# CloudEngineHub/PARC

Measured on AMD Instinct MI355X. Metric: env-steps/s, higher is better.
Workload: dtype f32; 1 GPU; full step (dynamics + obs/reward/done), 65536 envs total = 65536 per GPU, 5 bundled clips on a square blocky grid, reset of finished envs included; envs_per_gpu=65536, total_envs=65536, dynamics=True, parallelism=env-shard x1, launch=stream launches, library_abi=6

## Files before the change

### parc_amd/csrc/parc_env.hip

```cpp
#include <hip/hip_runtime.h>

#include <cmath>
#include <cstddef>
#include <cstdio>
#include <cstring>
#include <memory>
#include <new>
#include <string>
#include <type_traits>
#include <vector>

#include "../../include/parc_env.h"
#include "parc_common.hpp"
#include "parc_math.hpp"
#include "parc_rowmap.hpp"
#include "parc_lanetab.hpp"
#include "parc_dynamics.hpp"
#include "parc_dynamics_coop.hpp"
#include "parc_dynamics_wave.hpp"

using namespace parc;

#define REC_F4 32
#define REC_Q_POS 15
#define REC_Q_CONTACT 16
#define REC_Q_VEL 20

struct HierTables {
    float lt[16][3];
    float lr[16][4];
    int fk_paths[PARC_MAX_FK_PATHS][PARC_MAX_FK_DEPTH];
    int key_ids[8];
    int key_slot[16];
    int parent[16];
    int jtype[16];
    int dof_idx[16];
    float axis[16][4];
};
#define HIER_STAGED_WORDS ((int)(offsetof(HierTables, parent) / 4))

#define TILE_MAX_CELLS 320

struct DevTables {
    HierTables h;
    float tstep[8];
    float joint_err_w[16];
    float dof_err_w[PARC_MAX_DOFS];
    float contact_w[16];
    float pose_term_dist[16];
    ParcLaneEntry lane[64];
};

struct StepParams {
    int N, B, J, D, K, S, R, M, T;
    int lds_wave_floats;
    int global_obs, off_char;
    int lr_identity;
    int obs_tar, obs_contact;
    int obs_dim, off_dofvel, off_key, off_tar, tar_w, off_tarc, off_cc, off_hf;
    float dt_f, episode_length, min_obs_h, max_obs_h;
    float pose_w, vel_w, root_pos_w, root_vel_w, key_pos_w;
    float root_pos_term_sq, root_rot_term;
    int early_term, pose_term, track_root, track_root_h, tracking, body_pos_from_fk, never_done;
    unsigned fall_mask;
    float term_h;
    const float *hf; int X, Y; float min_x, min_y, dx, dy; int tile_r;
    float rdx, rdy;
    float tstep[8];
    const float4 *records; const MotionMeta *meta; const float *motion_offsets; const float *env_offsets;
    const float *ray_points; const DevTables *tables;
    unsigned char *ema_code;
    unsigned *stamp_out;
    float4 *prep;
    ParcEnvBuffers buf;
};

__device__ __forceinline__ Q4 joint_dof_to_rot(int type, const float *axis4, const float *dof) {
    if (type == PARC_JOINT_HINGE) return axis_angle_to_quat(mk3(axis4[0], axis4[1], axis4[2]), dof[0]);
    if (type == PARC_JOINT_SPHERICAL) return exp_map_to_quat(mk3(dof[0], dof[1], dof[2]));
    return mk4(0.f, 0.f, 0.f, 1.f);
}

__device__ __forceinline__ void joint_rot_to_dof(int type, const float *axis4, Q4 q, float *out) {
// ... 69 lines not shown
#endif
#define MODE_STEP 0
#define MODE_OBS 1
#define ENVS_PER_BLOCK 4
#define WAVE_SYNC() asm volatile("" ::: "memory")
#define RAY_UNROLL 8

__device__ __forceinline__ float wave_sum(float v) {
#pragma unroll
    for (int off = 32; off >= 1; off >>= 1) v = v + __shfl_xor(v, off, 64);
    return v;
}

template <int CTRL>
__device__ __forceinline__ float dpp_f32(float v) {
    return __int_as_float(__builtin_amdgcn_update_dpp(0, __float_as_int(v), CTRL, 0xf, 0xf, false));
}
__device__ __forceinline__ float row_sum16(float v) {
    v = v + dpp_f32<0x128>(v);
    v = v + dpp_f32<0x124>(v);
    v = v + dpp_f32<0x122>(v);
    v = v + dpp_f32<0x121>(v);
    return v;
}
__device__ __forceinline__ float lane_value(float v, int l) { return __int_as_float(__builtin_amdgcn_readlane(__float_as_int(v), l)); }

template <int MODE, bool MIRROR, bool LOCALROOT = false, bool OBSVAR = false>
__global__ __launch_bounds__(256, 5) void k_env_post(const StepParams P, const int64_t *__restrict__ env_ids,
                                                 const int *__restrict__ env_ids32, const int *__restrict__ count_dev, int count,
                                                 unsigned long long *bump_calls) {
    extern __shared__ __align__(16) float s_obs_all[];
    __shared__ int s_tab_raw[HIER_STAGED_WORDS];
    const HierTables &s_tab = *reinterpret_cast<const HierTables *>(s_tab_raw);
    __shared__ float4 s_q_all[ENVS_PER_BLOCK][8][16];
    __shared__ float4 s_lq_all[ENVS_PER_BLOCK][2][16];
    __shared__ float4 s_fk_all[ENVS_PER_BLOCK][80];
    __shared__ float s_cdofv_all[ENVS_PER_BLOCK][PARC_MAX_DOFS];
    __shared__ float4 s_refvel_all[ENVS_PER_BLOCK][12];
    __shared__ float s_refct_all[ENVS_PER_BLOCK][16];
    __shared__ float s_cfn_all[ENVS_PER_BLOCK][16];
    __shared__ float s_sc_all[ENVS_PER_BLOCK][16];
#ifdef PARC_STAMPS
    __shared__ unsigned long long s_stamp_all[ENVS_PER_BLOCK][16];
#endif
    const int wv = __builtin_amdgcn_readfirstlane((int)(threadIdx.x >> 6));
    const int lane = threadIdx.x & 63;
    const bool GLOBALOBS = OBSVAR && P.global_obs != 0;
    const int oc = OBSVAR ? P.off_char : 0;
    const bool TAROBS = !OBSVAR || P.obs_tar != 0;
    const bool CONTACTOBS = !OBSVAR || P.obs_contact != 0;
    float *s_obs = s_obs_all + (size_t)wv * P.lds_wave_floats;
    float4 (*s_q)[16] = s_q_all[wv];
    float4 (*s_lq)[16] = s_lq_all[wv];
    float4 *s_fk = s_fk_all[wv];
    float4 *s_cbp = s_lq[0];
    float *s_cdofv = s_cdofv_all[wv];
    float4 *s_refvel = s_refvel_all[wv];
    float *s_refct = s_refct_all[wv], *s_cfn = s_cfn_all[wv];
#ifdef PARC_STAMPS
    unsigned long long *s_stamp = s_stamp_all[wv];
#endif
    float *s_tile = (float *)s_fk;
    float4 (*s_br)[16] = reinterpret_cast<float4 (*)[16]>(s_obs + ((P.off_tarc + 3) & ~3));

    if (MODE == MODE_OBS && bump_calls && blockIdx.x == 0 && threadIdx.x == 0) *bump_calls += 1ull;
    if (count_dev) count = *count_dev;
    const int it = blockIdx.x * ENVS_PER_BLOCK + wv;
    if (it >= count) return;
    int e = env_ids ? (int)env_ids[it] : (env_ids32 ? env_ids32[it] : it);
    e = __builtin_amdgcn_readfirstlane(e);
    STAMP(0);

    const int B = P.B, D = P.D, S = P.S, K = P.K, J = P.J;
    const DevTables *__restrict__ T = P.tables;

    float *orow = P.buf.obs + (size_t)e * P.obs_dim;

    constexpr int HW = HIER_STAGED_WORDS;
    constexpr int HN = (HW + 63) / 64;
    int tabreg[HN];
#pragma unroll
    for (int i = 0; i < HN; ++i) { const int w = lane + 64 * i; tabreg[i] = w < HW ? ((const int *)&T->h)[w] : 0; }
    unsigned lt[PARC_LANETAB_WORDS];
    {
        static_assert(sizeof(ParcLaneEntry) == sizeof(uint4), "one 16-byte load per lane");
        const uint4 l0 = *reinterpret_cast<const uint4 *>(T->lane + lane);
        lt[0] = l0.x; lt[1] = l0.y; lt[2] = l0.z; lt[3] = l0.w;
// ... 24 lines not shown
    const float time = P.dt_f * (float)ts;
    const float mt = time + toff;
    const MotionMeta meta = P.meta[mid];
    const float eox = P.env_offsets[3 * e + 0], eoy = P.env_offsets[3 * e + 1], eoz = P.env_offsets[3 * e + 2];
    const float *mo = P.motion_offsets + 2 * ((size_t)mid * P.T + tid);
    const float offx = mo[0] - eox, offy = mo[1] - eoy;
    const float *crp = P.buf.char_root_pos + 3 * (size_t)e;
    const float *crr = P.buf.char_root_rot + 4 * (size_t)e;
    const V3 root_pos = mk3(crp[0], crp[1], crp[2]);
    const Q4 root_rot = mk4(crr[0], crr[1], crr[2], crr[3]);
    const float gx = root_pos.x + eox, gy = root_pos.y + eoy, gz = root_pos.z + eoz;

    Blend myb;
    {
        const int sid = lane & 7;
        float t = mt;
#pragma unroll
        for (int q = 0; q < PARC_MAX_TAR_STEPS; ++q) t = (sid - 1 == q) ? mt + P.tstep[q] : t;
        myb = frame_blend(meta, t);
    }
    const int last_frame = meta.start + meta.nframes - 1;
    float4 fA[2], fB[2];
    Blend bl[2];
#pragma unroll
    for (int p = 0; p < 2; ++p) {
        const int src4 = (int)parc_lt_src4(lt, p);
        bl[p].b = __int_as_float(__builtin_amdgcn_ds_bpermute(src4, __float_as_int(myb.b)));
        bl[p].i0 = __builtin_amdgcn_ds_bpermute(src4, myb.i0);
        bl[p].i1 = min(bl[p].i0 + 1, last_frame);
        const unsigned slot = parc_lt_row_slot(lt, p);
        fA[p] = P.records[(size_t)bl[p].i0 * REC_F4 + slot];
        fB[p] = P.records[(size_t)bl[p].i1 * REC_F4 + slot];
    }
    const int nvel = 2 + (D + 3) / 4;
    const int src4c = (int)parc_lt_src4(lt, 2);
    const float cblend = __int_as_float(__builtin_amdgcn_ds_bpermute(src4c, __float_as_int(myb.b)));
    const int b2i0 = __builtin_amdgcn_ds_bpermute(src4c, myb.i0), b2i1 = min(b2i0 + 1, last_frame);
    const float4 cA = P.records[(size_t)b2i0 * REC_F4 + parc_lt_cv_slot0(lt)];
    const float4 cB = P.records[(size_t)b2i1 * REC_F4 + parc_lt_cv_slot1(lt)];
    static_assert(64 * PARC_LANETAB_TILE_CELLS == TILE_MAX_CELLS && TILE_MAX_CELLS * sizeof(float) == sizeof(s_fk_all[0]), "the five tile stores of a lane stay inside s_fk");
    const int tr = P.tile_r, TW = 2 * tr + 1;
    const int ox = min(max(cell_index(gx, P.min_x, P.dx) - tr, -(1 << 22)), 1 << 22), oy = min(max(cell_index(gy, P.min_y, P.dy) - tr, -(1 << 22)), 1 << 22);
    float tilev[5];
#pragma unroll
    for (int i = 0; i < 5; ++i) {
        const int cx = min(max(ox + (int)parc_lt_cell_a(lt, i), 0), P.X - 1), cy = min(max(oy + (int)parc_lt_cell_b(lt, i), 0), P.Y - 1);
        tilev[i] = P.hf[(size_t)cx * P.Y + cy];
    }

    const float ch = __shfl(prepq.x, 0, 64), sh = __shfl(prepq.y, 0, 64);
    const Q4 hinv = mk4(0.f, 0.f, __shfl(prepq.z, 0, 64), __shfl(prepq.w, 0, 64));
#pragma unroll
    for (int i = 0; i < HN; ++i) { const int w = lane + 64 * i; if (w < HW) s_tab_raw[w] = tabreg[i]; }
    if (lane < D) {
        s_cdofv[lane] = dofv;
        s_obs[P.off_dofvel + lane] = dofv;
    }
    if (OBSVAR && oc && lane == 29) s_obs[0] = root_pos.z;
    if (role == PARC_LT_ROLE_ROOT_VEL || role == PARC_LT_ROLE_ROOT_ANG_VEL) {
        const V3 r = GLOBALOBS ? mk3(aux0, aux1, aux2) : quat_rotate(hinv, mk3(aux0, aux1, aux2));
        const int o = oc + (role == PARC_LT_ROLE_ROOT_VEL ? 6 : 9);
        s_obs[o + 0] = r.x; s_obs[o + 1] = r.y; s_obs[o + 2] = r.z;
    }
    if (role == PARC_LT_ROLE_FORCE) {
        const float n = norm3(mk3(aux0, aux1, aux2));
        if (CONTACTOBS) orow[P.off_cc + (lane - 32)] = n > 1e-5f ? 1.f : 0.f;
        s_cfn[lane - 32] = fminf(n, 1.0f);
    }
#pragma unroll
    for (int i = 0; i < 5; ++i) s_tile[lane + 64 * i] = tilev[i];
    WAVE_SYNC();
    STAMP(1);

    {
        float *hrow = orow + P.off_hf;
        float *hmirror = MIRROR && P.buf.ray_hfs ? P.buf.ray_hfs + (size_t)e * P.R : nullptr;
        for (int base = 0; base < P.R; base += 64 * RAY_UNROLL) {
            if (base > 0) {
#pragma unroll
                for (int i = 0; i < RAY_UNROLL; ++i) { const int r = base + lane + 64 * i; rayp[i] = r < P.R ? ((const float2 *)P.ray_points)[r] : make_float2(0.f, 0.f); }
            }
            const float tlox = (float)ox, thix = (float)(ox + TW - 1), tloy = (float)oy, thiy = (float)(oy + TW - 1);
            if (tr >= 0) {
                int tix[RAY_UNROLL];
#pragma unroll
                for (int i = 0; i < RAY_UNROLL; ++i) {
                    tix[i] = 0;
                    if (base + 64 * i < P.R) {
                        const float px = (rayp[i].x * ch - rayp[i].y * sh) + gx;
                        const float py = (rayp[i].x * sh + rayp[i].y * ch) + gy;
                        const int a = (int)fminf(fmaxf(cell_float_rcp(px, P.min_x, P.dx, P.rdx), tlox), thix) - ox;
                        const int bq = (int)fminf(fmaxf(cell_float_rcp(py, P.min_y, P.dy, P.rdy), tloy), thiy) - oy;
                        tix[i] = a * TW + bq;
                    }
                    asm volatile("" : "+v"(tix[i]));
                }
// ... 1 lines not shown
#pragma unroll
                for (int i = 0; i < RAY_UNROLL; ++i) hv[i] = s_tile[tix[i]];
#pragma unroll
                for (int i = 0; i < RAY_UNROLL; ++i) {
                    const int r = base + lane + 64 * i;
                    if (r < P.R) {
                        float h = hv[i] - gz;
                        h = fminf(fmaxf(h, P.min_obs_h), P.max_obs_h);
                        hrow[r] = h;
                        if (hmirror) hmirror[r] = h;
                    }
                }
            } else {
#pragma unroll
                for (int i = 0; i < RAY_UNROLL; ++i) {
                    const int r = base + lane + 64 * i;
                    if (r < P.R) {
                        const float px = (rayp[i].x * ch - rayp[i].y * sh) + gx;
                        const float py = (rayp[i].x * sh + rayp[i].y * ch) + gy;
                        const int ix = cell_index_rcp(px, P.min_x, P.dx, P.rdx), iy = cell_index_rcp(py, P.min_y, P.dy, P.rdy);
                        const int cx = min(max(ix, 0), P.X - 1), cy = min(max(iy, 0), P.Y - 1);
                        float h = P.hf[(size_t)cx * P.Y + cy] - gz;
                        h = fminf(fmaxf(h, P.min_obs_h), P.max_obs_h);
                        hrow[r] = h;
                        if (hmirror) hmirror[r] = h;
                    }
                }
            }
        }
    }
    STAMP(2);

    static_assert(2 * (PARC_MAX_BODIES - 2) <= PARC_ROWMAP_JOINTS_A, "the joints of rows 0 and 1 must fit into pass A");
    auto row_pass = [&](auto root_tag, const int itm, const float4 A, const float4 Bv, const float bb) {
        constexpr bool ROOT = decltype(root_tag)::value;
        if (itm < 0) return;
        const int r = itm >> 4, i = itm & 15;
        const bool is_rot = ROOT && i == 0, is_pos = ROOT && i == 15;
        const bool row0 = ROOT && r == 0, row1 = ROOT && r == 1;
        float4 res = make_float4(0.f, 0.f, 0.f, 1.f);
        if (row0) {
            if (is_rot) res = root_rot;
            else if (is_pos) res = make_float4(root_pos.x, root_pos.y, root_pos.z, 0.f);
            else res = prepq;
        } else {
            if (is_pos) {
                const float a = 1.0f - bb;
                res.x = a * A.x + bb * Bv.x;
                res.y = a * A.y + bb * Bv.y;
                res.z = a * A.z + bb * Bv.z;
                res.w = 0.f;
                if (meta.loop == PARC_LOOP_WRAP) {
                    float t = mt;
#pragma unroll
                    for (int q = 0; q < PARC_MAX_TAR_STEPS; ++q) t = (r - 2 == q) ? mt + P.tstep[q] : t;
                    const float ph = floorf(t / meta.length);
                    res.x = res.x + ph * meta.dx; res.y = res.y + ph * meta.dy; res.z = res.z + ph * meta.dz;
                }
                res.x = res.x + offx;
                res.y = res.y + offy;
            } else {
                res = slerp_rr(A, Bv, bb);
            }
        }
        if (!is_rot && !is_pos) {
            const Q4 lq = P.lr_identity ? res : quat_mul(mk4(s_tab.lr[i][0], s_tab.lr[i][1], s_tab.lr[i][2], s_tab.lr[i][3]), res);
            if (row0 || row1) { s_lq[r][i] = lq; s_q[r][i] = res; } else s_q[r][i] = lq;
        } else {
            s_q[r][i] = res;
        }
        if (row1) {
            if (MIRROR && is_rot && P.buf.ref_root_rot) *(float4 *)(P.buf.ref_root_rot + 4 * (size_t)e) = res;
            if (MIRROR && !is_rot && !is_pos && P.buf.ref_joint_rot) *(float4 *)(P.buf.ref_joint_rot + 4 * ((size_t)e * J + i - 1)) = res;
            if (MIRROR && is_pos && P.buf.ref_root_pos) {
                float *o = P.buf.ref_root_pos + 3 * (size_t)e;
                o[0] = res.x; o[1] = res.y; o[2] = res.z;
            }
        } else if (row0 || TAROBS) {
            const int base = row0 ? 0 : P.off_tar + (r - 2) * P.tar_w;
            if (!is_pos) {
                const Q4 qq = (is_rot && !GLOBALOBS) ? quat_mul(hinv, res) : res;
                float tn[6];
                quat_to_tan_norm(qq, tn);
                const int o = row0 ? oc + (is_rot ? 0 : 12 + 6 * (i - 1)) : base + 3 + 6 * i;
#pragma unroll
                for (int c = 0; c < 6; ++c) s_obs[o + c] = tn[c];
            } else if (!row0) {
                const V3 rpd = mk3(res.x - root_pos.x, res.y - root_pos.y, res.z - root_pos.z);
                const V3 rpo = GLOBALOBS ? rpd : quat_rotate(hinv, rpd);
                s_obs[base + 0] = rpo.x; s_obs[base + 1] = rpo.y; s_obs[base + 2] = rpo.z;
            }
        }
    };
    row_pass(std::true_type(), item[0], fA[0], fB[0], bl[0].b);
    row_pass(std::false_type(), item[1], fA[1], fB[1], bl[1].b);
    if (lane < 4 * (1 + S)) {
        const int s = lane >> 2, c = lane & 3;
        const float b = cblend, a = 1.0f - b;
        const float v[4] = {a * cA.x + b * cB.x, a * cA.y + b * cB.y, a * cA.z + b * cB.z, a * cA.w + b * cB.w};
#pragma unroll
        for (int k = 0; k < 4; ++k) {
            const int bd = 4 * c + k;
            if (bd < B) {
                if (s == 0) {
                    s_refct[bd] = v[k];
                    if (MIRROR && P.buf.ref_contacts) P.buf.ref_contacts[(size_t)e * B + bd] = v[k];
                } else if (TAROBS && CONTACTOBS) {
                    orow[P.off_tarc + (s - 1) * B + bd] = v[k];
                }
            }
        }
    } else if (lane >= 32 && lane < 32 + nvel) {
        const int c = lane - 32;
        s_refvel[c] = cA;
        if (MIRROR && c == 0 && P.buf.ref_root_vel) { float *o = P.buf.ref_root_vel + 3 * (size_t)e; o[0] = cA.x; o[1] = cA.y; o[2] = cA.z; }
        if (MIRROR && c == 1 && P.buf.ref_root_ang_vel) { float *o = P.buf.ref_root_ang_vel + 3 * (size_t)e; o[0] = cA.x; o[1] = cA.y; o[2] = cA.z; }
        if (MIRROR && c >= 2 && P.buf.ref_dof_vel) {
            const float vv[4] = {cA.x, cA.y, cA.z, cA.w};
            for (int k = 0; k < 4; ++k) { const int d = 4 * (c - 2) + k; if (d < D) P.buf.ref_dof_vel[(size_t)e * D + d] = vv[k]; }
        }
    }
    float bpx = 0.f, bpy = 0.f, bpz = 0.f;
    if (!P.body_pos_from_fk && lane < B) {
        const float *src = P.buf.char_body_pos + 3 * ((size_t)e * B + lane);
        bpx = src[0]; bpy = src[1]; bpz = src[2];
    }
    WAVE_SYNC();
    STAMP(3);

    {
        const int k = lane >> 3, c = lane & 7;
        if (k < 2 + S) {
            Q4 prot = s_q[k][0];
            const float4 *jq = k < 2 ? s_lq[k] : s_q[k];
            const float4 pp = s_q[k][15];
            V3 ppos = mk3(pp.x, pp.y, pp.z);
            if (c == 0 && k < 2) {
                s_fk[k * 16] = make_float4(ppos.x, ppos.y, ppos.z, 0.f);
                if (MIRROR && P.tracking) s_br[k][0] = prot;
            }
            int b = s_tab.fk_paths[c][0];
#pragma unroll 1
            for (int d = 0; d < PARC_MAX_FK_DEPTH && b >= 0; ++d) {
                const int nb = d + 1 < PARC_MAX_FK_DEPTH ? s_tab.fk_paths[c][d + 1] : -1;
                const V3 wt = quat_rotate(prot, mk3(s_tab.lt[b][0], s_tab.lt[b][1], s_tab.lt[b][2]));
                ppos = mk3(ppos.x + wt.x, ppos.y + wt.y, ppos.z + wt.z);
                if (nb >= 0 || (MIRROR && P.tracking)) prot = quat_mul(prot, jq[b]);
                if (k < 2) {
                    s_fk[k * 16 + b] = make_float4(ppos.x, ppos.y, ppos.z, 0.f);
                    if (MIRROR && P.tracking) s_br[k][b] = prot;
                } else {
                    const int slot = s_tab.key_slot[b];
                    if (slot >= 0) s_fk[32 + (k - 2) * 8 + slot] = make_float4(ppos.x, ppos.y, ppos.z, 0.f);
                }
                b = nb;
            }
        }
    }
    WAVE_SYNC();
    if (lane < B) s_cbp[lane] = P.body_pos_from_fk ? s_fk[lane] : make_float4(bpx, bpy, bpz, 0.f);
    STAMP(4);

    if (lane < 8 * (1 + S)) {
        const int row = lane >> 3, kk = lane & 7;
        if (kk < K) {
            if (row == 0) {
                const float4 kp = s_fk[s_tab.key_ids[kk]];
                const V3 rd = mk3(kp.x - root_pos.x, kp.y - root_pos.y, kp.z - root_pos.z);
                const V3 rl = GLOBALOBS ? rd : quat_rotate(hinv, rd);
                const int o = P.off_key + 3 * kk;
                s_obs[o] = rl.x; s_obs[o + 1] = rl.y; s_obs[o + 2] = rl.z;
            } else if (TAROBS) {
                const int r = row + 1;
                const float4 kp = s_fk[32 + (r - 2) * 8 + s_tab.key_slot[s_tab.key_ids[kk]]], trp = s_q[r][15];
                const V3 rd = mk3(kp.x - trp.x, kp.y - trp.y, kp.z - trp.z);
                const int tb = P.off_tar + (r - 2) * P.tar_w, o = tb + 3 + 6 * B + 3 * kk;
                if (GLOBALOBS) {
                    s_obs[o] = rd.x; s_obs[o + 1] = rd.y; s_obs[o + 2] = rd.z;
                } else {
                    const V3 rl = quat_rotate(hinv, rd);
                    s_obs[o] = rl.x + s_obs[tb]; s_obs[o + 1] = rl.y + s_obs[tb + 1]; s_obs[o + 2] = rl.z + s_obs[tb + 2];
                }
            }
        }
    }
    STAMP(5);

    if (MODE == MODE_STEP) {
        {
            float *sc = s_sc_all[wv];
            bool fc = false;
            if (P.fall_mask != 0u && lane >= 32 && lane < 32 + B && !((P.fall_mask >> (lane - 32)) & 1u))
                fc = fabsf(aux0) > 0.1f || fabsf(aux1) > 0.1f || fabsf(aux2) > 0.1f;
            const bool fcany = __ballot(fc) != 0ull;
            if (lane == 30) { sc[5] = aux0; sc[6] = aux1; sc[7] = aux2; }
            if (lane == 31) { sc[8] = aux0; sc[9] = aux1; sc[10] = aux2; }
            if (lane == 0) {
                sc[0] = time; sc[1] = mt; sc[2] = __int_as_float(ts); sc[3] = meta.length; sc[4] = __int_as_float(meta.loop);
                sc[11] = fcany ? 1.f : 0.f; sc[12] = eox; sc[13] = eoy; sc[14] = __int_as_float(e);
            }
        }
        asm volatile("s_waitcnt lgkmcnt(0)\n\ts_barrier" ::: "memory");
        const int nact = min(ENVS_PER_BLOCK, count - (int)blockIdx.x * ENVS_PER_BLOCK);
        int owner = blockIdx.x & (ENVS_PER_BLOCK - 1);
        if (owner >= nact) owner = 0;
        if (wv == owner) {
            const int j = lane >> 4, i = lane & 15, rowbase = lane & 48;
            const bool valid = j < nact;
            const int jj = valid ? j : 0;
            const float4 (*q)[16] = s_q_all[jj];
            const float4 *fk = s_fk_all[jj];
            const float4 *cbp = s_lq_all[jj][0];
            const float *scj = s_sc_all[jj];
            const float4 rp4 = q[0][15], trp = q[1][15];
            float dang = 0.f, vpose = 0.f;
            Q4 hinv_c = mk4(0.f, 0.f, 0.f, 1.f), hinv_r = hinv_c;
            if (LOCALROOT) {
                hinv_c = heading_quat_inv(calc_heading(q[0][0]));
                hinv_r = heading_quat_inv(calc_heading(q[1][0]));
            }
            if (i <= J) {
                const int slot = i < J ? 1 + i : 0;
                if (LOCALROOT) {
                    Q4 qa = q[0][slot], qb = q[1][slot];
                    if (i == J) { qa = quat_mul(hinv_c, qa); qb = quat_mul(hinv_r, qb); }
                    dang = quat_diff_angle(qa, qb);
                } else {
                    dang = quat_diff_angle(q[0][slot], q[1][slot]);
                }
                if (i < J) vpose = T->joint_err_w[i] * dang * dang;
            }
            float vs[4] = {0.f, 0.f, 0.f, 0.f};
#pragma unroll
            for (int pss = 0; pss < (PARC_MAX_DOFS + 15) / 16; ++pss) {
                if (16 * pss < D) {
                    const int d = 16 * pss + i;
                    float v = 0.f;
                    if (d < D) {
                        const float dv = ((const float *)s_refvel_all[jj])[8 + d] - s_cdofv_all[jj][d];
                        v = T->dof_err_w[d] * dv * dv;
                    }
                    vs[pss] = row_sum16(v);
                }
            }
// ... 21 lines not shown
                vct = T->contact_w[i] * cr;
            }
            bool bad = false;
            if (i >= 1 && i < B) {
                const float4 bp = cbp[i], b0 = cbp[0], tp = fk[16 + i], t0 = fk[16];
                const float dx = (tp.x - t0.x) - (bp.x - b0.x);
                const float dy = (tp.y - t0.y) - (bp.y - b0.y);
                const float dz = (tp.z - t0.z) - (bp.z - b0.z);
                const float lim = T->pose_term_dist[i - 1];
                bad = (dx * dx + dy * dy + dz * dz) > lim * lim;
            }
            const bool pose_fail_any = ((unsigned)(__ballot(bad) >> rowbase) & 0xffffu) != 0u;
            bool fallen = false;
            if (P.fall_mask != 0u) {
                bool fh = false;
                if (i < B && !((P.fall_mask >> i) & 1u)) {
                    const float4 bp = cbp[i];
                    const int ix = min(max(cell_index(bp.x + scj[12], P.min_x, P.dx), 0), P.X - 1), iy = min(max(cell_index(bp.y + scj[13], P.min_y, P.dy), 0), P.Y - 1);
                    fh = bp.z < P.hf[(size_t)ix * P.Y + iy] + P.term_h;
                }
                fallen = scj[11] != 0.f && ((unsigned)(__ballot(fh) >> rowbase) & 0xffffu) != 0u;
            }
            const float root_rot_angle = __shfl(dang, rowbase + J, 64);
            const float pose_err = __shfl(row_sum16(vpose), rowbase, 64), csum = __shfl(row_sum16(vct), rowbase, 64), key_err = __shfl(row_sum16(vkey), rowbase, 64);
            const float vel_err = __shfl((vs[0] + vs[1]) + (vs[2] + vs[3]), rowbase, 64);

            const float time_j = scj[0], mt_j = scj[1], mlen_j = scj[3];
            const int ts_j = __float_as_int(scj[2]), mloop_j = __float_as_int(scj[4]), e_j = __float_as_int(scj[14]);
            float rdx = trp.x - rp4.x, rdy = trp.y - rp4.y, rdz = trp.z - rp4.z;
            if (!P.track_root) { rdx = 0.f; rdy = 0.f; }
            if (!P.track_root_h) rdz = 0.f;
            const float root_pos_err = rdx * rdx + rdy * rdy + rdz * rdz;
            const float4 tv = s_refvel_all[jj][0], tav = s_refvel_all[jj][1];
            const float rre = root_rot_angle * root_rot_angle;
            float rve, rave;
            if (LOCALROOT) {
                const V3 tv3 = quat_rotate(hinv_r, mk3(tv.x, tv.y, tv.z)), tav3 = quat_rotate(hinv_r, mk3(tav.x, tav.y, tav.z));
                const V3 rv3 = quat_rotate(hinv_c, mk3(scj[5], scj[6], scj[7])), rav3 = quat_rotate(hinv_c, mk3(scj[8], scj[9], scj[10]));
                float d0 = tv3.x - rv3.x, d1 = tv3.y - rv3.y, d2 = tv3.z - rv3.z;
                rve = d0 * d0 + d1 * d1 + d2 * d2;
                d0 = tav3.x - rav3.x; d1 = tav3.y - rav3.y; d2 = tav3.z - rav3.z;
                rave = d0 * d0 + d1 * d1 + d2 * d2;
            } else {
                float d0 = tv.x - scj[5], d1 = tv.y - scj[6], d2 = tv.z - scj[7];
                rve = d0 * d0 + d1 * d1 + d2 * d2;
                d0 = tav.x - scj[8]; d1 = tav.y - scj[9]; d2 = tav.z - scj[10];
                rave = d0 * d0 + d1 * d1 + d2 * d2;
            }
            float earg = -0.25f * pose_err;
            earg = i == 1 ? -0.01f * vel_err : earg;
            earg = i == 2 ? -5.0f * (root_pos_err + 0.1f * rre) : earg;
            earg = i == 3 ? -1.0f * (rve + 0.1f * rave) : earg;
            earg = i == 4 ? -10.0f * key_err : earg;
            const float eval = expf(earg);
            const float pose_r = __shfl(eval, rowbase, 64), vel_r = __shfl(eval, rowbase + 1, 64), root_pose_r = __shfl(eval, rowbase + 2, 64),
                        root_vel_r = __shfl(eval, rowbase + 3, 64), key_pos_r = __shfl(eval, rowbase + 4, 64);
            float rew = P.pose_w * pose_r + P.vel_w * vel_r + P.root_pos_w * root_pose_r + P.root_vel_w * root_vel_r + P.key_pos_w * key_pos_r;
            const float contact_pen = (OBSVAR && P.obs_contact == 0) ? 0.f : csum / (float)B;
            rew = rew + contact_pen;
            int done = PARC_DONE_NULL;
            if (time_j >= P.episode_length) done = PARC_DONE_TIME;
            if (P.early_term) {
                bool failed = fallen;
                if (P.pose_term) {
                    bool pf = pose_fail_any;
                    if (P.track_root) {
                        const float4 b0 = cbp[0], t0 = fk[16];
                        const float ex = b0.x - t0.x, ey = b0.y - t0.y, ez = b0.z - t0.z;
                        pf = pf || (ex * ex + ey * ey + ez * ez) > P.root_pos_term_sq;
                        pf = pf || fabsf(root_rot_angle) > P.root_rot_term;
                    }
                    failed = failed || pf;
                }
                if (!(time_j > 1e-5f)) failed = false;
                if (failed) done = PARC_DONE_FAIL;
            }
            const bool motion_end = (mt_j >= mlen_j) && (mloop_j != PARC_LOOP_WRAP);
            unsigned char code = 0;
            if (done != PARC_DONE_NULL || motion_end) code = (done == PARC_DONE_FAIL) ? 1 : 2;
// ... 803 lines not shown
    }
    for (int p = 0; p < PARC_MAX_FK_PATHS; ++p)
        for (int d = 0; d < PARC_MAX_FK_DEPTH; ++d) {
            t.h.fk_paths[p][d] = m.fk_paths[p][d];
            if (m.fk_paths[p][d] >= B) return fail(PARC_ERR_INVALID, "fk_paths entry out of range");
        }
    const float dt_f = (float)cfg->control_dt;
    for (int s = 0; s < S; ++s) t.tstep[s] = dt_f * (float)cfg->tar_obs_steps[s];
    for (int k = 0; k < K; ++k) {
        if (cfg->key_body_ids[k] < 0 || cfg->key_body_ids[k] >= B) return fail(PARC_ERR_INVALID, "key body id out of range");
        t.h.key_ids[k] = cfg->key_body_ids[k];
        if (t.h.key_slot[cfg->key_body_ids[k]] < 0) t.h.key_slot[cfg->key_body_ids[k]] = k;
    }
    for (int j = 0; j < J; ++j) { t.joint_err_w[j] = cfg->joint_err_w[j]; t.pose_term_dist[j] = cfg->pose_termination_dist[j]; }
    for (int d = 0; d < D; ++d) t.dof_err_w[d] = cfg->dof_err_w[d];
    for (int b = 0; b < B; ++b) t.contact_w[b] = cfg->contact_weights[b];

    StepParams &sp = e->sp;
    memset(&sp, 0, sizeof(sp));
    sp.N = e->N; sp.B = B; sp.J = J; sp.D = D; sp.K = K; sp.S = S; sp.R = R;
    sp.global_obs = cfg->global_obs; sp.off_char = cfg->global_root_height_obs ? 1 : 0;
    sp.off_dofvel = sp.off_char + 12 + 6 * J;
    sp.off_key = sp.off_dofvel + D;
    sp.off_tar = sp.off_key + 3 * K;
    sp.tar_w = 3 + 6 + 6 * J + 3 * K;
    e->row_mul = parc_rowmap_mul(B);
    if (!parc_rowmap_mul_ok(B, e->row_mul)) return fail(PARC_ERR_INVALID, "internal: row item multiplier");
    if (!parc_lanetab_fill(t.lane, B, S, D, R, -1, e->row_mul, 0u)) return fail(PARC_ERR_INVALID, "internal: lane table");
    sp.lr_identity = 1;
    for (int b = 0; b < B; ++b)
        if (!(cfg->model.local_rotation[b][0] == 0.f && cfg->model.local_rotation[b][1] == 0.f && cfg->model.local_rotation[b][2] == 0.f && cfg->model.local_rotation[b][3] == 1.f)) sp.lr_identity = 0;
    sp.obs_tar = cfg->enable_tar_obs != 0; sp.obs_contact = cfg->use_contact_info != 0;
    sp.off_tarc = sp.off_tar + (sp.obs_tar ? S * sp.tar_w : 0);
    sp.off_cc = sp.off_tarc + (sp.obs_tar && sp.obs_contact ? S * B : 0);
    sp.off_hf = sp.off_cc + (sp.obs_contact ? B : 0);
    sp.obs_dim = sp.off_hf + R;
    e->obs_dim = sp.obs_dim;
    for (int q = 0; q < S; ++q) sp.tstep[q] = dt_f * (float)cfg->tar_obs_steps[q];
    sp.dt_f = dt_f; sp.episode_length = cfg->episode_length; sp.min_obs_h = cfg->min_obs_h; sp.max_obs_h = cfg->max_obs_h;
    sp.pose_w = cfg->pose_w; sp.vel_w = cfg->vel_w; sp.root_pos_w = cfg->root_pos_w; sp.root_vel_w = cfg->root_vel_w; sp.key_pos_w = cfg->key_pos_w;
    sp.root_pos_term_sq = (float)((double)cfg->root_pos_termination_dist * (double)cfg->root_pos_termination_dist);
    sp.root_rot_term = cfg->root_rot_termination_angle;
    sp.early_term = cfg->enable_early_termination; sp.pose_term = cfg->pose_termination; sp.track_root = cfg->track_root;
    sp.track_root_h = cfg->track_root_h; sp.tracking = cfg->report_tracking_error; sp.body_pos_from_fk = cfg->body_pos_from_fk;
    sp.fall_mask = cfg->contact_body_mask & ((1u << B) - 1u); sp.term_h = cfg->termination_height;

    DeviceArena &mem = e->mem;
    const long long N = e->N;
    PARC_TRY(mem.alloc(e->d_tab, 1, &t));
    PARC_TRY(mem.alloc_fill(e->d_prep, 16 * N));
    PARC_TRY(mem.alloc(e->d_ray, 2 * R, cfg->ray_points_host));
    PARC_TRY(mem.alloc(e->d_env_off, 3 * N, cfg->env_offsets_host));
    PARC_TRY(mem.alloc_fill(e->d_ema, (N + 1023) / 1024 * 1024));
    PARC_TRY(mem.alloc_fill(e->d_done_list, N));
    PARC_TRY(mem.alloc_fill(e->d_done_key, N));
    PARC_TRY(mem.alloc_fill(e->d_chunk_count, 1024));
    PARC_TRY(mem.alloc_fill(e->d_reset_count, 2));
    PARC_TRY(mem.alloc_fill(e->d_reset_calls, 1));
    PARC_TRY(mem.alloc_fill(e->d_scratch_jr, 4 * J * N));
    {
        RenderGeoms rg;
        memset(&rg, 0, sizeof(rg));
        const ParcDynamicsParams &dp = cfg->dynamics;
        for (int g = 0; g < dp.num_geoms && g < PARC_MAX_GEOMS; ++g) {
            if (dp.geom_body[g] < 0 || dp.geom_body[g] >= B || dp.geom_type[g] < PARC_GEOM_BOX || dp.geom_type[g] > PARC_GEOM_CAPSULE) continue;
            const int n = rg.n++;
// ... 1078 lines not shown
```

### parc_amd/csrc/parc_lanetab.hpp

```cpp
#pragma once

#include "parc_rowmap.hpp"

#define PARC_LANETAB_WORDS 4
#define PARC_LANETAB_TILE_CELLS 5
#define PARC_LANETAB_RAY_SLOTS 8

#define PARC_LT_ROLE_NONE 0
#define PARC_LT_ROLE_ROOT_VEL 1
#define PARC_LT_ROLE_ROOT_ANG_VEL 2
#define PARC_LT_ROLE_FORCE 3

struct alignas(16) ParcLaneEntry { unsigned w[PARC_LANETAB_WORDS]; };

PARC_ROWMAP_HD unsigned parc_lt_bits(unsigned w, int lo, int n) { return (w >> lo) & ((1u << n) - 1u); }
PARC_ROWMAP_HD int parc_lt_item(const unsigned *w, int pass) { return (int)(w[0] << (pass == 0 ? 24 : 16)) >> 24; }
PARC_ROWMAP_HD unsigned parc_lt_src4(const unsigned *w, int which) { return parc_lt_bits(w[1], 5 * which, 5); }
PARC_ROWMAP_HD unsigned parc_lt_row_slot(const unsigned *w, int pass) { return parc_lt_bits(w[1], 15 + 4 * pass, 4); }
PARC_ROWMAP_HD unsigned parc_lt_cv_slot0(const unsigned *w) { return parc_lt_bits(w[1], 23, 5); }
PARC_ROWMAP_HD unsigned parc_lt_cv_slot1(const unsigned *w) { return 16u + parc_lt_bits(w[0], 16, 2); }
PARC_ROWMAP_HD unsigned parc_lt_role(const unsigned *w) { return parc_lt_bits(w[1], 28, 2); }
PARC_ROWMAP_HD unsigned parc_lt_force_off(const unsigned *w) { return parc_lt_bits(w[0], 18, 6); }
PARC_ROWMAP_HD unsigned parc_lt_dof(const unsigned *w) { return parc_lt_bits(w[0], 24, 6); }
PARC_ROWMAP_HD unsigned parc_lt_cell(const unsigned *w, int i) { return i < 3 ? parc_lt_bits(w[2], 10 * i, 10) : parc_lt_bits(w[3], 10 * (i - 3), 10); }
// ... 16 lines not shown
    if (20 + nvel > 32) return false;
    for (int lane = 0; lane < 64; ++lane) {
        unsigned *w = tab[lane].w;
        for (int i = 0; i < PARC_LANETAB_WORDS; ++i) w[i] = 0u;
        const int item[2] = {parc_rowmap_item<true>(lane, B, 2 + S, row_mul), parc_rowmap_item<false>(lane, B, 2 + S, row_mul)};
        w[0] = ((unsigned)item[0] & 0xffu) | (((unsigned)item[1] & 0xffu) << 8);
        for (int p = 0; p < 2; ++p) {
            const int it = item[p] > 0 ? item[p] : 0, r = it >> 4;
            w[1] |= (unsigned)(4 * (r > 1 ? r - 1 : 0)) << (5 * p);
            w[1] |= (unsigned)(it & 15) << (15 + 4 * p);
        }
        const bool contact = lane < 4 * (1 + S), vel = !contact && lane >= 32 && lane < 32 + nvel;
        w[1] |= (unsigned)(4 * (contact ? lane >> 2 : 0)) << 10;
        w[1] |= (unsigned)(contact ? 16 + (lane & 3) : vel ? 20 + (lane - 32) : 16) << 23;
        w[0] |= (unsigned)(contact ? lane & 3 : 0) << 16;
        const bool force = lane >= 32 && lane < 32 + B;
        w[1] |= (unsigned)(lane == 30 ? PARC_LT_ROLE_ROOT_VEL : lane == 31 ? PARC_LT_ROLE_ROOT_ANG_VEL : force ? PARC_LT_ROLE_FORCE : PARC_LT_ROLE_NONE) << 28;
        w[0] |= (unsigned)(force ? 3 * (lane - 32) : 0) << 18;
        w[0] |= (unsigned)(lane < D ? lane : D - 1) << 24;
        for (int i = 0; i < PARC_LANETAB_TILE_CELLS; ++i) {
            const int idx = lane + 64 * i;
            if (idx >= ncell) continue;
            const unsigned a = ((unsigned)idx * tile_mul) >> 16, bq = (unsigned)idx - a * (unsigned)TW;
            if (a > 31u || bq > 31u) return false;
            w[i < 3 ? 2 : 3] |= (a | bq << 5) << (10 * (i < 3 ? i : i - 3));
            w[3] |= 1u << (20 + i);
        }
        unsigned nray = 0;
        for (int i = 0; i < PARC_LANETAB_RAY_SLOTS; ++i) nray += lane + 64 * i < R ? 1u : 0u;
        w[3] |= nray << 25;
    }
    return true;
}
```

Measured before the change: 101.7 million env-steps/s.

## Table-drive heading rotations into one packed per-lane pass over a unified LDS block

Gathers every heading-frame rotation (target root offsets, root velocities, key-body positions, target key positions) into a single table-driven pass. Each lane reads src/sub/dst byte offsets from a precomputed per-lane table, and the target root offset is added through a ds_bpermute. The q, fk and root-velocity LDS arrays are merged into one contiguous block so those offsets can be encoded. Contact/velocity reference writes are also driven by the table, including a vectorized float4 store of ref contacts. This is meant to remove scattered divergent branches and serialized quat_rotate work. The cost is extra table loads and a bpermute dependency.

Measured after the change: 102.9 million env-steps/s, median of 6. +1.1%, better.

```diff
diff --git a/parc_amd/csrc/parc_env.hip b/parc_amd/csrc/parc_env.hip
--- a/parc_amd/csrc/parc_env.hip
+++ b/parc_amd/csrc/parc_env.hip
@@ -49,6 +49,7 @@
     float contact_w[16];
     float pose_term_dist[16];
     ParcLaneEntry lane[64];
+    ParcHrotEntry hrot[64];
 };
 
 struct StepParams {
@@ -184,12 +185,11 @@
     extern __shared__ __align__(16) float s_obs_all[];
     __shared__ int s_tab_raw[HIER_STAGED_WORDS];
     const HierTables &s_tab = *reinterpret_cast<const HierTables *>(s_tab_raw);
-    __shared__ float4 s_q_all[ENVS_PER_BLOCK][8][16];
+    __shared__ float4 s_blk_all[ENVS_PER_BLOCK][PARC_HROT_BLOCK_F4];
     __shared__ float4 s_lq_all[ENVS_PER_BLOCK][2][16];
-    __shared__ float4 s_fk_all[ENVS_PER_BLOCK][80];
     __shared__ float s_cdofv_all[ENVS_PER_BLOCK][PARC_MAX_DOFS];
     __shared__ float4 s_refvel_all[ENVS_PER_BLOCK][12];
-    __shared__ float s_refct_all[ENVS_PER_BLOCK][16];
+    __shared__ __align__(16) float s_refct_all[ENVS_PER_BLOCK][16];
     __shared__ float s_cfn_all[ENVS_PER_BLOCK][16];
     __shared__ float s_sc_all[ENVS_PER_BLOCK][16];
 #ifdef PARC_STAMPS
@@ -202,9 +202,10 @@
     const bool TAROBS = !OBSVAR || P.obs_tar != 0;
     const bool CONTACTOBS = !OBSVAR || P.obs_contact != 0;
     float *s_obs = s_obs_all + (size_t)wv * P.lds_wave_floats;
-    float4 (*s_q)[16] = s_q_all[wv];
+    float4 (*s_q)[16] = reinterpret_cast<float4 (*)[16]>(s_blk_all[wv] + PARC_HROT_Q_F4);
     float4 (*s_lq)[16] = s_lq_all[wv];
-    float4 *s_fk = s_fk_all[wv];
+    float4 *s_fk = s_blk_all[wv] + PARC_HROT_FK_F4;
+    float4 *s_rv = s_blk_all[wv] + PARC_HROT_RV_F4;
     float4 *s_cbp = s_lq[0];
     float *s_cdofv = s_cdofv_all[wv];
     float4 *s_refvel = s_refvel_all[wv];
@@ -295,13 +296,12 @@
         fA[p] = P.records[(size_t)bl[p].i0 * REC_F4 + slot];
         fB[p] = P.records[(size_t)bl[p].i1 * REC_F4 + slot];
     }
-    const int nvel = 2 + (D + 3) / 4;
     const int src4c = (int)parc_lt_src4(lt, 2);
     const float cblend = __int_as_float(__builtin_amdgcn_ds_bpermute(src4c, __float_as_int(myb.b)));
     const int b2i0 = __builtin_amdgcn_ds_bpermute(src4c, myb.i0), b2i1 = min(b2i0 + 1, last_frame);
     const float4 cA = P.records[(size_t)b2i0 * REC_F4 + parc_lt_cv_slot0(lt)];
     const float4 cB = P.records[(size_t)b2i1 * REC_F4 + parc_lt_cv_slot1(lt)];
-    static_assert(64 * PARC_LANETAB_TILE_CELLS == TILE_MAX_CELLS && TILE_MAX_CELLS * sizeof(float) == sizeof(s_fk_all[0]), "the five tile stores of a lane stay inside s_fk");
+    static_assert(64 * PARC_LANETAB_TILE_CELLS == TILE_MAX_CELLS && TILE_MAX_CELLS * sizeof(float) == (PARC_HROT_RV_F4 - PARC_HROT_FK_F4) * sizeof(float4), "the five tile stores of a lane stay inside s_fk");
     const int tr = P.tile_r, TW = 2 * tr + 1;
     const int ox = min(max(cell_index(gx, P.min_x, P.dx) - tr, -(1 << 22)), 1 << 22), oy = min(max(cell_index(gy, P.min_y, P.dy) - tr, -(1 << 22)), 1 << 22);
     float tilev[5];
@@ -320,11 +320,9 @@
         s_obs[P.off_dofvel + lane] = dofv;
     }
     if (OBSVAR && oc && lane == 29) s_obs[0] = root_pos.z;
-    if (role == PARC_LT_ROLE_ROOT_VEL || role == PARC_LT_ROLE_ROOT_ANG_VEL) {
-        const V3 r = GLOBALOBS ? mk3(aux0, aux1, aux2) : quat_rotate(hinv, mk3(aux0, aux1, aux2));
-        const int o = oc + (role == PARC_LT_ROLE_ROOT_VEL ? 6 : 9);
-        s_obs[o + 0] = r.x; s_obs[o + 1] = r.y; s_obs[o + 2] = r.z;
-    }
+    static_assert(PARC_LT_ROLE_ROOT_VEL == 1 && PARC_LT_ROLE_ROOT_ANG_VEL == 2 && PARC_HROT_RV_ZERO == 2, "s_rv slots");
+    if (role == PARC_LT_ROLE_ROOT_VEL || role == PARC_LT_ROLE_ROOT_ANG_VEL) s_rv[role - 1] = make_float4(aux0, aux1, aux2, 0.f);
+    if (lane == 29) s_rv[PARC_HROT_RV_ZERO] = make_float4(0.f, 0.f, 0.f, 0.f);
     if (role == PARC_LT_ROLE_FORCE) {
         const float n = norm3(mk3(aux0, aux1, aux2));
         if (CONTACTOBS) orow[P.off_cc + (lane - 32)] = n > 1e-5f ? 1.f : 0.f;
@@ -392,6 +390,11 @@
     STAMP(2);
 
     static_assert(2 * (PARC_MAX_BODIES - 2) <= PARC_ROWMAP_JOINTS_A, "the joints of rows 0 and 1 must fit into pass A");
+    unsigned hr[3];
+    {
+        const unsigned *h0 = T->hrot[lane].w;
+        hr[0] = h0[0]; hr[1] = h0[1]; hr[2] = h0[2];
+    }
     auto row_pass = [&](auto root_tag, const int itm, const float4 A, const float4 Bv, const float bb) {
         constexpr bool ROOT = decltype(root_tag)::value;
         if (itm < 0) return;
@@ -445,33 +448,30 @@
                 const int o = row0 ? oc + (is_rot ? 0 : 12 + 6 * (i - 1)) : base + 3 + 6 * i;
 #pragma unroll
                 for (int c = 0; c < 6; ++c) s_obs[o + c] = tn[c];
-            } else if (!row0) {
-                const V3 rpd = mk3(res.x - root_pos.x, res.y - root_pos.y, res.z - root_pos.z);
-                const V3 rpo = GLOBALOBS ? rpd : quat_rotate(hinv, rpd);
-                s_obs[base + 0] = rpo.x; s_obs[base + 1] = rpo.y; s_obs[base + 2] = rpo.z;
             }
         }
     };
     row_pass(std::true_type(), item[0], fA[0], fB[0], bl[0].b);
     row_pass(std::false_type(), item[1], fA[1], fB[1], bl[1].b);
-    if (lane < 4 * (1 + S)) {
-        const int s = lane >> 2, c = lane & 3;
+    const unsigned cvk = parc_hr_cv_kind(hr);
+    if (cvk == PARC_HR_CV_REF || cvk == PARC_HR_CV_TAR) {
         const float b = cblend, a = 1.0f - b;
         const float v[4] = {a * cA.x + b * cB.x, a * cA.y + b * cB.y, a * cA.z + b * cB.z, a * cA.w + b * cB.w};
-#pragma unroll
-        for (int k = 0; k < 4; ++k) {
-            const int bd = 4 * c + k;
-            if (bd < B) {
-                if (s == 0) {
-                    s_refct[bd] = v[k];
-                    if (MIRROR && P.buf.ref_contacts) P.buf.ref_contacts[(size_t)e * B + bd] = v[k];
-                } else if (TAROBS && CONTACTOBS) {
-                    orow[P.off_tarc + (s - 1) * B + bd] = v[k];
-                }
-            }
-        }
-    } else if (lane >= 32 && lane < 32 + nvel) {
-        const int c = lane - 32;
+        const int nk = (int)parc_hr_cv_n(hr);
+        if (cvk == PARC_HR_CV_REF) {
+            const int c = (int)parc_hr_cv_idx(hr);
+            *reinterpret_cast<float4 *>(s_refct + 4 * c) = make_float4(v[0], v[1], v[2], v[3]);
+            if (MIRROR && P.buf.ref_contacts) {
+#pragma unroll
+                for (int k = 0; k < 4; ++k) if (k < nk) P.buf.ref_contacts[(size_t)e * B + 4 * c + k] = v[k];
+            }
+        } else {
+            float *o = reinterpret_cast<float *>(reinterpret_cast<char *>(orow) + parc_hr_cv_off(hr));
+#pragma unroll
+            for (int k = 0; k < 4; ++k) if (k < nk) o[k] = v[k];
+        }
+    } else if (cvk == PARC_HR_CV_VEL) {
+        const int c = (int)parc_hr_cv_idx(hr);
         s_refvel[c] = cA;
         if (MIRROR && c == 0 && P.buf.ref_root_vel) { float *o = P.buf.ref_root_vel + 3 * (size_t)e; o[0] = cA.x; o[1] = cA.y; o[2] = cA.z; }
         if (MIRROR && c == 1 && P.buf.ref_root_ang_vel) { float *o = P.buf.ref_root_ang_vel + 3 * (size_t)e; o[0] = cA.x; o[1] = cA.y; o[2] = cA.z; }
@@ -521,28 +521,21 @@
     if (lane < B) s_cbp[lane] = P.body_pos_from_fk ? s_fk[lane] : make_float4(bpx, bpy, bpz, 0.f);
     STAMP(4);
 
-    if (lane < 8 * (1 + S)) {
-        const int row = lane >> 3, kk = lane & 7;
-        if (kk < K) {
-            if (row == 0) {
-                const float4 kp = s_fk[s_tab.key_ids[kk]];
-                const V3 rd = mk3(kp.x - root_pos.x, kp.y - root_pos.y, kp.z - root_pos.z);
-                const V3 rl = GLOBALOBS ? rd : quat_rotate(hinv, rd);
-                const int o = P.off_key + 3 * kk;
-                s_obs[o] = rl.x; s_obs[o + 1] = rl.y; s_obs[o + 2] = rl.z;
-            } else if (TAROBS) {
-                const int r = row + 1;
-                const float4 kp = s_fk[32 + (r - 2) * 8 + s_tab.key_slot[s_tab.key_ids[kk]]], trp = s_q[r][15];
-                const V3 rd = mk3(kp.x - trp.x, kp.y - trp.y, kp.z - trp.z);
-                const int tb = P.off_tar + (r - 2) * P.tar_w, o = tb + 3 + 6 * B + 3 * kk;
-                if (GLOBALOBS) {
-                    s_obs[o] = rd.x; s_obs[o + 1] = rd.y; s_obs[o + 2] = rd.z;
-                } else {
-                    const V3 rl = quat_rotate(hinv, rd);
-                    s_obs[o] = rl.x + s_obs[tb]; s_obs[o + 1] = rl.y + s_obs[tb + 1]; s_obs[o + 2] = rl.z + s_obs[tb + 2];
-                }
-            }
-        }
+    if (parc_hr_item(hr)) {
+        const char *blk = reinterpret_cast<const char *>(s_q);
+        const float *sp = reinterpret_cast<const float *>(blk + parc_hr_src(hr)), *sb = reinterpret_cast<const float *>(blk + parc_hr_sub(hr));
+        const V3 rd = mk3(sp[0] - sb[0], sp[1] - sb[1], sp[2] - sb[2]);
+        V3 rl = rd;
+        if (!GLOBALOBS) {
+            rl = quat_rotate(hinv, rd);
+            const int a4 = (int)parc_hr_add4(hr);
+            const float ax = __int_as_float(__builtin_amdgcn_ds_bpermute(a4, __float_as_int(rl.x)));
+            const float ay = __int_as_float(__builtin_amdgcn_ds_bpermute(a4, __float_as_int(rl.y)));
+            const float az = __int_as_float(__builtin_amdgcn_ds_bpermute(a4, __float_as_int(rl.z)));
+            if (parc_hr_adds(hr)) rl = mk3(rl.x + ax, rl.y + ay, rl.z + az);
+        }
+        float *o = reinterpret_cast<float *>(reinterpret_cast<char *>(s_obs) + parc_hr_dst(hr));
+        o[0] = rl.x; o[1] = rl.y; o[2] = rl.z;
     }
     STAMP(5);
 
@@ -553,8 +546,6 @@
             if (P.fall_mask != 0u && lane >= 32 && lane < 32 + B && !((P.fall_mask >> (lane - 32)) & 1u))
                 fc = fabsf(aux0) > 0.1f || fabsf(aux1) > 0.1f || fabsf(aux2) > 0.1f;
             const bool fcany = __ballot(fc) != 0ull;
-            if (lane == 30) { sc[5] = aux0; sc[6] = aux1; sc[7] = aux2; }
-            if (lane == 31) { sc[8] = aux0; sc[9] = aux1; sc[10] = aux2; }
             if (lane == 0) {
                 sc[0] = time; sc[1] = mt; sc[2] = __int_as_float(ts); sc[3] = meta.length; sc[4] = __int_as_float(meta.loop);
                 sc[11] = fcany ? 1.f : 0.f; sc[12] = eox; sc[13] = eoy; sc[14] = __int_as_float(e);
@@ -568,8 +559,8 @@
             const int j = lane >> 4, i = lane & 15, rowbase = lane & 48;
             const bool valid = j < nact;
             const int jj = valid ? j : 0;
-            const float4 (*q)[16] = s_q_all[jj];
-            const float4 *fk = s_fk_all[jj];
+            const float4 (*q)[16] = reinterpret_cast<const float4 (*)[16]>(s_blk_all[jj] + PARC_HROT_Q_F4);
+            const float4 *fk = s_blk_all[jj] + PARC_HROT_FK_F4;
             const float4 *cbp = s_lq_all[jj][0];
             const float *scj = s_sc_all[jj];
             const float4 rp4 = q[0][15], trp = q[1][15];
@@ -657,19 +648,20 @@
             if (!P.track_root_h) rdz = 0.f;
             const float root_pos_err = rdx * rdx + rdy * rdy + rdz * rdz;
             const float4 tv = s_refvel_all[jj][0], tav = s_refvel_all[jj][1];
+            const float4 cv = s_blk_all[jj][PARC_HROT_RV_F4 + 0], cav = s_blk_all[jj][PARC_HROT_RV_F4 + 1];
             const float rre = root_rot_angle * root_rot_angle;
             float rve, rave;
             if (LOCALROOT) {
                 const V3 tv3 = quat_rotate(hinv_r, mk3(tv.x, tv.y, tv.z)), tav3 = quat_rotate(hinv_r, mk3(tav.x, tav.y, tav.z));
-                const V3 rv3 = quat_rotate(hinv_c, mk3(scj[5], scj[6], scj[7])), rav3 = quat_rotate(hinv_c, mk3(scj[8], scj[9], scj[10]));
+                const V3 rv3 = quat_rotate(hinv_c, mk3(cv.x, cv.y, cv.z)), rav3 = quat_rotate(hinv_c, mk3(cav.x, cav.y, cav.z));
                 float d0 = tv3.x - rv3.x, d1 = tv3.y - rv3.y, d2 = tv3.z - rv3.z;
                 rve = d0 * d0 + d1 * d1 + d2 * d2;
                 d0 = tav3.x - rav3.x; d1 = tav3.y - rav3.y; d2 = tav3.z - rav3.z;
                 rave = d0 * d0 + d1 * d1 + d2 * d2;
             } else {
-                float d0 = tv.x - scj[5], d1 = tv.y - scj[6], d2 = tv.z - scj[7];
+                float d0 = tv.x - cv.x, d1 = tv.y - cv.y, d2 = tv.z - cv.z;
                 rve = d0 * d0 + d1 * d1 + d2 * d2;
-                d0 = tav.x - scj[8]; d1 = tav.y - scj[9]; d2 = tav.z - scj[10];
+                d0 = tav.x - cav.x; d1 = tav.y - cav.y; d2 = tav.z - cav.z;
                 rave = d0 * d0 + d1 * d1 + d2 * d2;
             }
             float earg = -0.25f * pose_err;
@@ -1539,6 +1531,8 @@
         if (!(cfg->model.local_rotation[b][0] == 0.f && cfg->model.local_rotation[b][1] == 0.f && cfg->model.local_rotation[b][2] == 0.f && cfg->model.local_rotation[b][3] == 1.f)) sp.lr_identity = 0;
     sp.obs_tar = cfg->enable_tar_obs != 0; sp.obs_contact = cfg->use_contact_info != 0;
     sp.off_tarc = sp.off_tar + (sp.obs_tar ? S * sp.tar_w : 0);
+    if (!parc_hrot_fill(t.hrot, B, S, D, K, t.h.key_ids, t.h.key_slot, sp.off_char, sp.off_key, sp.off_tar, sp.tar_w, sp.obs_tar, sp.obs_tar && sp.obs_contact, sp.global_obs, sp.off_tarc))
+        return fail(PARC_ERR_INVALID, "internal: heading-pass table");
     sp.off_cc = sp.off_tarc + (sp.obs_tar && sp.obs_contact ? S * B : 0);
     sp.off_hf = sp.off_cc + (sp.obs_contact ? B : 0);
     sp.obs_dim = sp.off_hf + R;
diff --git a/parc_amd/csrc/parc_lanetab.hpp b/parc_amd/csrc/parc_lanetab.hpp
--- a/parc_amd/csrc/parc_lanetab.hpp
+++ b/parc_amd/csrc/parc_lanetab.hpp
@@ -72,3 +72,78 @@
     }
     return true;
 }
+
+#define PARC_HROT_Q_F4 0
+#define PARC_HROT_FK_F4 128
+#define PARC_HROT_RV_F4 208
+#define PARC_HROT_RV_ZERO 2
+#define PARC_HROT_BLOCK_F4 212
+
+struct alignas(4) ParcHrotEntry { unsigned w[3]; };
+
+PARC_ROWMAP_HD unsigned parc_hr_src(const unsigned *w) { return parc_lt_bits(w[0], 0, 12); }
+PARC_ROWMAP_HD unsigned parc_hr_sub(const unsigned *w) { return parc_lt_bits(w[0], 16, 12); }
+PARC_ROWMAP_HD unsigned parc_hr_dst(const unsigned *w) { return parc_lt_bits(w[1], 0, 14); }
+PARC_ROWMAP_HD unsigned parc_hr_add4(const unsigned *w) { return parc_lt_bits(w[1], 16, 8); }
+PARC_ROWMAP_HD bool parc_hr_item(const unsigned *w) { return (w[1] >> 24 & 1u) != 0u; }
+PARC_ROWMAP_HD bool parc_hr_adds(const unsigned *w) { return (w[1] >> 25 & 1u) != 0u; }
+
+#define PARC_HR_CV_NONE 0
+#define PARC_HR_CV_REF 1
+#define PARC_HR_CV_TAR 2
+#define PARC_HR_CV_VEL 3
+PARC_ROWMAP_HD unsigned parc_hr_cv_off(const unsigned *w) { return parc_lt_bits(w[2], 0, 16); }
+PARC_ROWMAP_HD unsigned parc_hr_cv_n(const unsigned *w) { return parc_lt_bits(w[2], 16, 3); }
+PARC_ROWMAP_HD unsigned parc_hr_cv_kind(const unsigned *w) { return parc_lt_bits(w[2], 20, 2); }
+PARC_ROWMAP_HD unsigned parc_hr_cv_idx(const unsigned *w) { return parc_lt_bits(w[2], 24, 4); }
+
+inline bool parc_hrot_fill_cv(ParcHrotEntry *tab, int B, int S, int D, int off_tarc, int tar_contacts) {
+    if (B < 2 || B > 15 || S < 0 || S > 6 || D < 1 || D > 40) return false;
+    const int nvel = 2 + (D + 3) / 4;
+    for (int lane = 0; lane < 64; ++lane) {
+        unsigned &w = tab[lane].w[2];
+        w = 0u;
+        const int s = lane >> 2, c = lane & 3, nk = B - 4 * c < 0 ? 0 : B - 4 * c > 4 ? 4 : B - 4 * c;
+        if (lane < 4 * (1 + S)) {
+            if (nk == 0 || (s > 0 && !tar_contacts)) continue;
+            const int off = s > 0 ? 4 * (off_tarc + (s - 1) * B + 4 * c) : 0;
+            if (off >= (1 << 16)) return false;
+            w = (unsigned)off | (unsigned)nk << 16 | (unsigned)(s == 0 ? PARC_HR_CV_REF : PARC_HR_CV_TAR) << 20 | (unsigned)c << 24;
+        } else if (lane >= 32 && lane < 32 + nvel) {
+            if (lane - 32 > 11) return false;
+            w = (unsigned)PARC_HR_CV_VEL << 20 | (unsigned)(lane - 32) << 24;
+        }
+    }
+    return true;
+}
+
+inline bool parc_hrot_fill(ParcHrotEntry *tab, int B, int S, int D, int K, const int *key_ids, const int *key_slot, int oc, int off_key, int off_tar,
+                           int tar_w, int tar_obs, int tar_contacts, int global_obs, int nst) {
+    if (B < 2 || B > 15 || S < 0 || S > 6 || K < 0 || K > 8) return false;
+    for (int lane = 0; lane < 64; ++lane) tab[lane].w[0] = tab[lane].w[1] = 0u;
+    if (!parc_hrot_fill_cv(tab, B, S, D, nst, tar_contacts)) return false;
+    int n = 0;
+    bool ok = true;
+    auto put = [&](int src_f4, int sub_f4, int dst, int add_lane) {
+        if (n >= 64 || src_f4 < 0 || src_f4 >= PARC_HROT_BLOCK_F4 || sub_f4 < 0 || sub_f4 >= PARC_HROT_BLOCK_F4 || dst < 0 || dst + 3 > nst || 4 * dst >= (1 << 14)) { ok = false; return; }
+        tab[n].w[0] = (unsigned)(16 * src_f4) | (unsigned)(16 * sub_f4) << 16;
+        tab[n].w[1] = (unsigned)(4 * dst) | (unsigned)(add_lane >= 0 ? 4 * add_lane : 0) << 16 | 1u << 24 | (add_lane >= 0 ? 1u : 0u) << 25;
+        ++n;
+    };
+    const int root0 = PARC_HROT_Q_F4 + 15;
+    const int nroot = tar_obs ? S : 0;
+    for (int s = 0; s < nroot; ++s) put(PARC_HROT_Q_F4 + 16 * (2 + s) + 15, root0, off_tar + s * tar_w, -1);
+    put(PARC_HROT_RV_F4 + 0, PARC_HROT_RV_F4 + PARC_HROT_RV_ZERO, oc + 6, -1);
+    put(PARC_HROT_RV_F4 + 1, PARC_HROT_RV_F4 + PARC_HROT_RV_ZERO, oc + 9, -1);
+    for (int k = 0; k < K; ++k) {
+        if (key_ids[k] < 0 || key_ids[k] >= B) return false;
+        put(PARC_HROT_FK_F4 + key_ids[k], root0, off_key + 3 * k, -1);
+    }
+    for (int s = 0; s < nroot; ++s)
+        for (int k = 0; k < K; ++k) {
+            const int slot = key_slot[key_ids[k]];
+            if (slot < 0 || slot >= 8) return false;
+            put(PARC_HROT_FK_F4 + 32 + 8 * s + slot, PARC_HROT_Q_F4 + 16 * (2 + s) + 15, off_tar + s * tar_w + 3 + 6 * B + 3 * k, global_obs ? -1 : s);
+        }
+    return ok;
+}
```
